# daac-tools/daachorse

Hardware: NVIDIA H100
Metric: input GB/s scanned, find_overlapping_iter, 675k-pat bytewise (higher is better)
Workload: dtype u8

## Files before the change

### daachorse_b200/csrc/dev_scan.cu

```cuda
#include <cuda_runtime.h>

#include <unistd.h>

#include <algorithm>
#include <atomic>
#include <chrono>
#include <cstdio>
#include <cstdlib>
#include <cstring>
#include <memory>
#include <mutex>
#include <string>
#include <vector>

#include "dev_image.h"
#include "host.h"
#include "scan_lane.cuh"

namespace dach {


constexpr int kMaxThreads = 1024;
constexpr int kMaxDevices = 64;
constexpr uint32_t kRootBytes = 1024;
constexpr int64_t kDefaultDfPairs = 1 << 24;

template <int RK>
using SinkOf = typename std::conditional<
    RK == RK_COUNT, CountSink,
    typename std::conditional<
        RK == RK_FIRST || RK == RK_FIRST_STREAM, FirstSink,
        typename std::conditional<RK == RK_HIST, HistSink, typename std::conditional<RK == RK_DF, DfSink, Emitter>::type>::type>::type>::type;

template <bool CHARWISE, int MODE, class SINK>
__device__ __forceinline__ void scan_items(const ScanParams& P) {
    extern __shared__ __align__(16) unsigned char smem_raw[];
    uint32_t* s_root = reinterpret_cast<uint32_t*>(smem_raw);
    uint4* s_hot = reinterpret_cast<uint4*>(smem_raw + kRootBytes);
    for (uint32_t i = threadIdx.x; i < 256; i += blockDim.x) s_root[i] = P.root_table[i];
    for (uint32_t i = threadIdx.x; i < P.hot_n; i += blockDim.x) s_hot[i] = P.rec[i];
    __syncthreads();

    RecView V{P.rec, s_hot, P.hot_n, s_root};
    TextWin T;
    SINK E;
    for (;;) {
        const unsigned long long item = bump_u64(&P.ctrl->next_item);
        if (item >= P.n_items) break;
        const uint64_t o0 = P.offs[item], o1 = P.offs[item + 1];
        const uint32_t len = (uint32_t)(o1 - o0);
        T.open(P.text + o0);
        E.begin((uint32_t)item);
        if (MODE == M_LEFTMOST)
            scan_leftmost<CHARWISE>(P, V, T, E, len);
        else
            scan_standard<CHARWISE, MODE>(P, V, T, E, len);
        E.finish(P);
    }
}

template <bool CHARWISE, int MODE>
__global__ void __launch_bounds__(kMaxThreads, 1) k_scan(ScanParams P) {
    scan_items<CHARWISE, MODE, Emitter>(P);
}
template <bool CHARWISE, int MODE, int RK>
__global__ void __launch_bounds__(kMaxThreads, 1) k_scan_rk(ScanParams P) {
    scan_items<CHARWISE, MODE, SinkOf<RK>>(P);
}


__device__ __forceinline__ uint32_t smem_u32(const void* p) { return (uint32_t)__cvta_generic_to_shared(p); }

__device__ __forceinline__ void mbar_init(uint64_t* bar, uint32_t count) {
    asm volatile("mbarrier.init.shared::cta.b64 [%0], %1;" ::"r"(smem_u32(bar)), "r"(count) : "memory");
    asm volatile("fence.mbarrier_init.release.cluster;" ::: "memory");
}
__device__ __forceinline__ void mbar_expect_tx(uint64_t* bar, uint32_t bytes) {
// ... 83 lines not shown
            if (need) {
                const unsigned long long item = base + __popc(m & ((1u << lane) - 1u));
                if (item < n_items)
                    OPS::begin_item(L, P, Ev, E, item, nullptr);
                else
                    exhausted = true;
            }
        }
        if (!__any_sync(FULL, (L.fl & F_ACTIVE) != 0)) break;
        bool stop = false;
        while (!stop) {
            M::text_topup(L, Ev, nullptr);
            if (M::LEAN) {
#pragma unroll 1
                for (int k = 0; k < M::TOPUP; ++k) (void)M::step(L, Ev, nullptr);
                stop = __any_sync(FULL, (L.fl & (F_ACTIVE | M::IDLE)) == (F_ACTIVE | M::IDLE));
            } else if (M::LAZY) {
                bool waiting = false;
#pragma unroll 1
                for (int k = 0; k < M::TOPUP; ++k) {
                    const bool ok = M::step(L, Ev, nullptr);
                    waiting |= !ok;
                }
                stop = __any_sync(FULL, waiting && (L.fl & F_ACTIVE));
            } else {
#pragma unroll 1
                for (int k = 0; k < M::TOPUP; ++k) {
                    const bool ok = M::step(L, Ev, nullptr);
                    if (__any_sync(FULL, !ok && (L.fl & F_ACTIVE))) {
                        stop = true;
                        break;
                    }
                }
            }
        }
    }
    if constexpr (SINK::KIND == RK_HIST) {
        __syncthreads();
        for (uint32_t i = threadIdx.x; i < P.hist_smem; i += blockDim.x)
            if (E.s_cnt[i]) red_add_u64(P.slot_hist + i, E.s_cnt[i]);
    }
}

template <class M, class LANE, int MAXT, int MINB, bool HOT>
__global__ void __launch_bounds__(MAXT, MINB) k_scan_machine(ScanParams P) {
    if constexpr (M::QLEN)
        scan_machine<M, EventOps<M::ITER>, LANE, EventSink, HOT>(P);
    else
        scan_machine<M, M, LANE, Emitter, HOT>(P);
}
template <class M, class LANE, int MODE, int RK, bool HOT>
__global__ void __launch_bounds__(1024, 1) k_scan_machine_rk(ScanParams P) {
    scan_machine<M, SinkOps<M, MODE, RK>, LANE, SinkOf<RK>, HOT>(P);
}

template <int MODE, int MAXT, bool HOT>
__global__ void __launch_bounds__(MAXT, 1) k_scan_duo(ScanParams P) {
    using M = StdMachine3<MODE>;
    extern __shared__ __align__(128) unsigned char smem_raw[];
    uint4* s_hot = reinterpret_cast<uint4*>(smem_raw);
    QEntry* s_queue = reinterpret_cast<QEntry*>(smem_raw + (HOT ? (size_t)P.hot_entries * 16 : 0));
    __shared__ __align__(8) uint64_t s_bar;
    if (HOT) {
        if (threadIdx.x == 0) mbar_init(&s_bar, 1);
        __syncthreads();
        if (threadIdx.x == 0) {
            const uint32_t hot_bytes = P.hot_entries * 16u;
            mbar_expect_tx(&s_bar, hot_bytes);
            for (uint32_t off = 0; off < hot_bytes; off += 32768u)
                tma_bulk_g2s(reinterpret_cast<unsigned char*>(s_hot) + off, reinterpret_cast<const unsigned char*>(P.crec) + off,
                             min(32768u, hot_bytes - off), &s_bar);
        }
    }
    const StdEnv Ev0{P.crec, s_hot, smem_u32(s_hot), HOT ? P.hot_entries : 0u, P.opos_tab, P.text_end, P.text_lo, P.root_base, P.root_opos ? CF_OUT : 0u,
                     s_queue + threadIdx.x, blockDim.x, 0u, P.mapper, P.mapper_len, ld_u4(P.crec + D_ROOT)};
    StdEnv Ev1 = Ev0;
    Ev1.q = s_queue + (size_t)LANE_Q * blockDim.x + threadIdx.x;
    const unsigned FULL = 0xffffffffu;
    const unsigned lane = threadIdx.x & 31u;
    const unsigned lt = (1u << lane) - 1u;
    Lane3 L0, L1;
    L0.fl = L1.fl = M::IDLE;
    L0.qn = L1.qn = 0;
    Emitter E0, E1;
    E0.begin(0);
    E1.begin(0);
    bool exhausted = false;
    const unsigned long long n_items = P.n_items_dev ? *P.n_items_dev : P.n_items;
    constexpr uint32_t WAIT = F_ACTIVE | F3_STOP;
    if (HOT) mbar_wait(&s_bar, 0);
    for (;;) {
        if (L0.fl & F_ACTIVE) M::drain(L0, Ev0, P, E0);
        if (L1.fl & F_ACTIVE) M::drain(L1, Ev1, P, E1);
        if ((L0.fl & (F_ACTIVE | F_DONE)) == (F_ACTIVE | F_DONE)) {
            E0.finish(P);
            M::finish_item(L0, P);
            L0.fl = M::IDLE;
        }
        if ((L1.fl & (F_ACTIVE | F_DONE)) == (F_ACTIVE | F_DONE)) {
            E1.finish(P);
            M::finish_item(L1, P);
            L1.fl = M::IDLE;
        }
        const bool need0 = !(L0.fl & F_ACTIVE) && !exhausted, need1 = !(L1.fl & F_ACTIVE) && !exhausted;
        const unsigned m0 = __ballot_sync(FULL, need0), m1 = __ballot_sync(FULL, need1);
        if (m0 | m1) {
// ... 614 lines not shown
            }
        if (pinned) cudaFreeHost(pinned);
        pinned = nullptr;
        if (offs_stage) cudaFreeHost(offs_stage);
        offs_stage = nullptr;
        offs_stage_bytes = 0;
        for (int i = 0; i < 4; ++i)
            if (ev[i]) {
                cudaEventDestroy(ev[i]);
                ev[i] = nullptr;
            }
        for (int i = 0; i < 2; ++i)
            if (ev_push[i]) {
                cudaEventDestroy(ev_push[i]);
                ev_push[i] = nullptr;
            }
        if (ev_scanned) cudaEventDestroy(ev_scanned);
        if (ev_placed) cudaEventDestroy(ev_placed);
        ev_scanned = ev_placed = nullptr;
        if (stream) cudaStreamDestroy(stream);
        stream = nullptr;
    }
};

}

struct dach_dev {
    int device = 0;
    bool charwise = false;
    uint8_t match_kind = 0;
    uint32_t n_slots = 0, root_opos = 0, mapper_len = 0, max_pattern_len = 0;
    bool segmentable = false;
    uint32_t n_outputs = 0, max_value = 0, n_cslots = 0;
    size_t image_bytes = 0;
    int sm_count = 0;
    size_t smem_optin = 0;
    uint4* d_rec = nullptr;
    uint4* d_outputs = nullptr;
    uint32_t* d_root = nullptr;
    uint4* d_crec = nullptr;
    uint32_t* d_opos = nullptr;
    uint32_t* d_id_in = nullptr;
    uint32_t* d_id_out = nullptr;
    uint32_t hot_slots = 0;
    uint32_t root_base = 0;
    uint32_t* d_mapper = nullptr;
    void* image_base = nullptr;
    size_t image_alloc = 0;
    std::mutex mu;
    Workspace ws;
    static constexpr int kSlots = 4;
    Workspace slot[kSlots];
    int64_t opt_slice_mib = 64;
    int64_t opt_hot_entries = 6144;
    int64_t opt_hist_smem = 1024;
    int64_t opt_df_pairs = kDefaultDfPairs;
    int64_t opt_slice_ramp = 1;
    int64_t opt_tail_seg = 0;
    int64_t opt_gather_ordered = 1;
    int64_t opt_gather_u = 4;
    int64_t opt_reserve_sms = 0;
    int64_t opt_smem_pad_kib = 0;
    int64_t opt_seg_len = 0;
    int64_t opt_hot_records = 0;
    int64_t opt_threads = 1024;
    int64_t opt_ctas_per_sm = 1;
    int64_t opt_l2_hints = 2;
    int64_t opt_kernel = 3;
    std::atomic<uint64_t> launches{0};
    cudaEvent_t ev_ref = nullptr;
    double last_scan_ms = 0, last_total_ms = 0;
    uint64_t last_h2d = 0, last_d2h = 0;
    DevBuf df_tab[2], df_list[2], df_n, df_acc;
    uint32_t df_mask = 0, df_limit = 0;
    bool df_clean = false;
    uint64_t last_df_windows = 0, last_df_rescans = 0;
    std::atomic<int> refs{1};
};

struct dach_job {
    dach_dev* d = nullptr;
    Workspace W;
    uint64_t out_cap = ~0ull;
};

namespace {

struct DeviceGuard {
    int prev = -1;
    bool ok = false;
    explicit DeviceGuard(int dev) {
        if (cudaGetDevice(&prev) != cudaSuccess) prev = -1;
        ok = cuda_ok(cudaSetDevice(dev), "cudaSetDevice");
        if (!ok) cudaGetLastError();
    }
    ~DeviceGuard() {
        if (prev >= 0) cudaSetDevice(prev);
    }
};

template <bool CW, int MODE>
cudaError_t launch_scan_t(const ScanParams& P, int grid, int threads, size_t smem, cudaStream_t st) {
    static bool attr_done[kMaxDevices] = {};
    int dev = 0;
    cudaGetDevice(&dev);
    if (dev < 0 || dev >= kMaxDevices || !attr_done[dev]) {
        cudaError_t e = cudaFuncSetAttribute(k_scan<CW, MODE>, cudaFuncAttributeMaxDynamicSharedMemorySize, 226 * 1024);
// ... 22 lines not shown
cudaError_t launch_std_modes(int mode, const ScanParams& P, int grid, int threads, size_t smem, cudaStream_t st) {
    switch (mode) {
        case M_FIND: return launch_machine_t<M<M_FIND>, LANE, MAXT, MINB, HOT>(P, grid, threads, smem, st);
        case M_NO_SUFFIX: return launch_machine_t<M<M_NO_SUFFIX>, LANE, MAXT, MINB, HOT>(P, grid, threads, smem, st);
        case M_OVERLAPPING: return launch_machine_t<M<M_OVERLAPPING>, LANE, MAXT, MINB, HOT>(P, grid, threads, smem, st);
    }
    return cudaErrorInvalidValue;
}

cudaError_t launch_std(int which, int mode, const ScanParams& P, int grid, int threads, size_t smem, cudaStream_t st,
                       bool dense) {
    if (which >= 3) {
        if (P.hot_entries)
            return dense ? launch_std_modes<StdMachine3, Lane3, 768, 2, true>(mode, P, grid, threads, smem, st)
                         : launch_std_modes<StdMachine3, Lane3, 1024, 1, true>(mode, P, grid, threads, smem, st);
        return dense ? launch_std_modes<StdMachine3, Lane3, 768, 2, false>(mode, P, grid, threads, smem, st)
                     : launch_std_modes<StdMachine3, Lane3, 1024, 1, false>(mode, P, grid, threads, smem, st);
    }
    if (which == 2)
        return dense ? launch_std_modes<StdMachine2, Lane2, 768, 2, false>(mode, P, grid, threads, smem, st)
                     : launch_std_modes<StdMachine2, Lane2, 1024, 1, false>(mode, P, grid, threads, smem, st);
    return dense ? launch_std_modes<StdMachine, LaneStd, 768, 2, false>(mode, P, grid, threads, smem, st)
                 : launch_std_modes<StdMachine, LaneStd, 1024, 1, false>(mode, P, grid, threads, smem, st);
}

template <int MODE, int MAXT, bool HOT>
cudaError_t launch_duo_t(const ScanParams& P, int grid, int threads, size_t smem, cudaStream_t st) {
    static bool attr_done[kMaxDevices] = {};
    int dev = 0;
    cudaGetDevice(&dev);
    if (dev < 0 || dev >= kMaxDevices || !attr_done[dev]) {
        cudaError_t e = cudaFuncSetAttribute(k_scan_duo<MODE, MAXT, HOT>, cudaFuncAttributeMaxDynamicSharedMemorySize, 226 * 1024);
        if (e != cudaSuccess) return e;
        if (dev >= 0 && dev < kMaxDevices) attr_done[dev] = true;
    }
    k_scan_duo<MODE, MAXT, HOT><<<grid, threads, smem, st>>>(P);
    return cudaGetLastError();
}
template <int MAXT, bool HOT>
cudaError_t launch_duo_m(int mode, const ScanParams& P, int grid, int threads, size_t smem, cudaStream_t st) {
    switch (mode) {
        case M_FIND: return launch_duo_t<M_FIND, MAXT, HOT>(P, grid, threads, smem, st);
        case M_NO_SUFFIX: return launch_duo_t<M_NO_SUFFIX, MAXT, HOT>(P, grid, threads, smem, st);
        case M_OVERLAPPING: return launch_duo_t<M_OVERLAPPING, MAXT, HOT>(P, grid, threads, smem, st);
    }
    return cudaErrorInvalidValue;
}
cudaError_t launch_duo(int mode, const ScanParams& P, int grid, int threads, size_t smem, cudaStream_t st) {
    if (threads > 768)
        return P.hot_entries ? launch_duo_m<1024, true>(mode, P, grid, threads, smem, st) : launch_duo_m<1024, false>(mode, P, grid, threads, smem, st);
    return P.hot_entries ? launch_duo_m<768, true>(mode, P, grid, threads, smem, st) : launch_duo_m<768, false>(mode, P, grid, threads, smem, st);
}

cudaError_t launch_cw(int mode, const ScanParams& P, int grid, int threads, size_t smem, cudaStream_t st) {
    switch (mode) {
        case M_FIND: return launch_machine_t<CwMachine<M_FIND>, LaneCw, 1024, 1, false>(P, grid, threads, smem, st);
        case M_OVERLAPPING: return launch_machine_t<CwMachine<M_OVERLAPPING>, LaneCw, 1024, 1, false>(P, grid, threads, smem, st);
        case M_NO_SUFFIX: return launch_machine_t<CwMachine<M_NO_SUFFIX>, LaneCw, 1024, 1, false>(P, grid, threads, smem, st);
        default: return launch_machine_t<CwMachine<M_LEFTMOST>, LaneCw, 1024, 1, false>(P, grid, threads, smem, st);
    }
}

cudaError_t launch_lm(const ScanParams& P, int grid, int threads, size_t smem, cudaStream_t st) {
    return launch_machine_t<LmMachine, LaneLm, 1024, 1, false>(P, grid, threads, smem, st);
}

cudaError_t launch_scan(bool cw, int mode, const ScanParams& P, int grid, int threads, size_t smem, cudaStream_t st) {
    switch ((cw ? 4 : 0) + mode) {
        case 0: return launch_scan_t<false, M_FIND>(P, grid, threads, smem, st);
        case 1: return launch_scan_t<false, M_OVERLAPPING>(P, grid, threads, smem, st);
        case 2: return launch_scan_t<false, M_NO_SUFFIX>(P, grid, threads, smem, st);
        case 3: return launch_scan_t<false, M_LEFTMOST>(P, grid, threads, smem, st);
        case 4: return launch_scan_t<true, M_FIND>(P, grid, threads, smem, st);
        case 5: return launch_scan_t<true, M_OVERLAPPING>(P, grid, threads, smem, st);
        case 6: return launch_scan_t<true, M_NO_SUFFIX>(P, grid, threads, smem, st);
        case 7: return launch_scan_t<true, M_LEFTMOST>(P, grid, threads, smem, st);
    }
    return cudaErrorInvalidValue;
}

template <class M, class LANE, int MODE, int RK, bool HOT>
cudaError_t launch_rk_t(const ScanParams& P, int grid, int threads, size_t smem, cudaStream_t st) {
    static bool attr_done[kMaxDevices] = {};
    int dev = 0;
    cudaGetDevice(&dev);
    if (dev < 0 || dev >= kMaxDevices || !attr_done[dev]) {
        cudaError_t e = cudaFuncSetAttribute(k_scan_machine_rk<M, LANE, MODE, RK, HOT>, cudaFuncAttributeMaxDynamicSharedMemorySize, 226 * 1024);
        if (e != cudaSuccess) return e;
        if (dev >= 0 && dev < kMaxDevices) attr_done[dev] = true;
    }
    k_scan_machine_rk<M, LANE, MODE, RK, HOT><<<grid, threads, smem, st>>>(P);
    return cudaGetLastError();
}
template <bool CW, int MODE, int RK>
cudaError_t launch_scan_rk_t(const ScanParams& P, int grid, int threads, size_t smem, cudaStream_t st) {
    static bool attr_done[kMaxDevices] = {};
    int dev = 0;
    cudaGetDevice(&dev);
    if (dev < 0 || dev >= kMaxDevices || !attr_done[dev]) {
        cudaError_t e = cudaFuncSetAttribute(k_scan_rk<CW, MODE, RK>, cudaFuncAttributeMaxDynamicSharedMemorySize, 226 * 1024);
        if (e != cudaSuccess) return e;
        if (dev >= 0 && dev < kMaxDevices) attr_done[dev] = true;
    }
    k_scan_rk<CW, MODE, RK><<<grid, threads, smem, st>>>(P);
    return cudaGetLastError();
}
// ... 63 lines not shown
        return DACH_INVALID_ARGUMENT;
    }
    const bool lm = is_leftmost(d->match_kind);
    if ((mode == DACH_LEFTMOST_FIND) != lm) {
        set_error(lm ? "Error: match_kind must be standard." : "Error: match_kind must be leftmost.");
        return DACH_MATCH_KIND_MISMATCH;
    }
    return DACH_OK;
}

bool install_policies(int hints) {
    unsigned long long* d_pol = nullptr;
    unsigned long long h_pol[3] = {0, 0, 0};
    if (!cuda_ok(cudaMalloc(reinterpret_cast<void**>(&d_pol), 24), "cudaMalloc policies")) return false;
    k_make_policies<<<1, 1>>>(d_pol, hints);
    bool ok = cuda_ok(cudaMemcpy(h_pol, d_pol, 24, cudaMemcpyDeviceToHost), "read policies");
    cudaFree(d_pol);
    return ok && cuda_ok(cudaMemcpyToSymbol(c_l2pol, h_pol, 24), "install policies");
}

ScanParams image_params(const dach_dev* d, const uint8_t* d_text, const uint8_t* text_lo, const uint8_t* text_end,
                        const uint64_t* d_offs, uint64_t n) {
    ScanParams P;
    memset(&P, 0, sizeof(P));
    P.rec = d->d_rec;
    P.outputs = d->d_outputs;
    P.root_table = d->d_root;
    P.crec = d->d_crec;
    P.opos_tab = d->d_opos;
    P.root_base = d->root_base;
    P.mapper = d->d_mapper;
    P.mapper_len = d->mapper_len;
    P.n_slots = d->n_slots;
    P.id_in = d->d_id_in;
    P.id_out = d->d_id_out;
    P.root_opos = d->root_opos;
    P.text = d_text;
    P.text_lo = text_lo;
    P.text_end = text_end;
    P.offs = d_offs;
    P.n_items = n;
    return P;
}

size_t plan_smem(const dach_dev* d, ScanParams& P, bool v1, bool std3, int threads, int ctas_per_sm, int queue_sets,
                 uint32_t hist_smem = 0) {
    const size_t smem_budget = std::min<size_t>(d->smem_optin, 226 * 1024) / ctas_per_sm - (ctas_per_sm > 1 ? 1024 : 0);
    size_t smem;
    if (v1) {
        const size_t queues = (size_t)LANE_Q * threads * sizeof(QEntry) * queue_sets + (size_t)hist_smem * 4;
        uint64_t want = 0;
        if (std3 && d->opt_hot_entries != 0 && smem_budget > queues + 512) {
            want = std::min<uint64_t>(d->hot_slots, (smem_budget - queues - 512) / 16);
            if (d->opt_hot_entries > 0) want = std::min<uint64_t>(want, (uint64_t)d->opt_hot_entries);
            want &= ~uint64_t(255);
        }
        smem = (size_t)want * 16 + queues;
        if (d->opt_smem_pad_kib > 0) smem = std::min<size_t>(smem + ((size_t)d->opt_smem_pad_kib << 10), smem_budget);
        P.hot_n = 0;
        P.hot_entries = (uint32_t)want;
    } else {
        uint64_t hot = smem_budget > kRootBytes ? (smem_budget - kRootBytes) / 16 : 0;
        if (d->opt_hot_records >= 0) hot = std::min<uint64_t>(hot, (uint64_t)d->opt_hot_records);
        hot = std::min<uint64_t>(hot, d->n_slots);
        P.hot_n = (uint32_t)hot;
        smem = kRootBytes + (size_t)hot * 16;
    }
    return smem;
}

void enqueue_seg_table(dach_dev* d, Workspace& W, const uint64_t* d_offs, uint64_t n, uint32_t seg_len, uint32_t seg_from,
                       ScanParams& P, cudaStream_t st) {
    unsigned long long* tiles = static_cast<unsigned long long*>(W.tiles.p);
    unsigned long long* seg_first = static_cast<unsigned long long*>(W.seg_first.p);
    const unsigned hb = (unsigned)((n + 255) / 256), hb1 = (unsigned)((n + 1 + 255) / 256);
    const uint64_t nt = (n + kScanTile - 1) / kScanTile;
    uint32_t* nseg = static_cast<uint32_t*>(W.nseg.p);
    k_seg_count<<<hb, 256, 0, st>>>(d_offs, n, seg_len, seg_from, nseg, P.ctrl);
    k_offsets_tile_sums<1><<<(unsigned)nt, kScanThreads, 0, st>>>(nseg, n, tiles);
    k_offsets_scan_tiles<<<1, kScanThreads, 0, st>>>(tiles, nt);
    k_offsets_apply<1><<<(unsigned)nt, kScanThreads, 0, st>>>(nseg, n, tiles, seg_first);
    k_seg_fill<<<hb1, 256, 0, st>>>(seg_first, nseg, n, seg_len, static_cast<uint32_t*>(W.item_hay.p),
                                    static_cast<uint32_t*>(W.item_beg.p), static_cast<unsigned long long*>(W.n_items_dev.p));
    d->launches += 5;
    P.item_hay = static_cast<const uint32_t*>(W.item_hay.p);
    P.item_beg = static_cast<const uint32_t*>(W.item_beg.p);
    P.n_items_dev = static_cast<const unsigned long long*>(W.n_items_dev.p);
    P.seg_len = seg_len;
    P.seg_from = seg_from;
    P.warm = d->max_pattern_len ? d->max_pattern_len - 1 : 0;
}

int enqueue_scan(dach_dev* d, Workspace& W, int mode, const uint8_t* d_text, const uint8_t* text_lo, const uint8_t* text_end,
                 uint64_t text_bytes, const uint64_t* d_offs, uint64_t n, uint64_t cap_matches, cudaStream_t st,
                 uint32_t* d_state_io = nullptr) {
    W.refused = false;
    if (n > 0xfffffff0ull) {
        set_error("too many haystacks in one batch (max 2^32-16)");
        return DACH_INVALID_ARGUMENT;
    }
    if (W.job_open) cudaStreamWaitEvent(st, W.ev_placed, 0);
    W.job_n = n;
    W.job_cap = cap_matches;
    W.job_items = n;
    W.job_seg = false;
    W.job_ordered = false;
    W.job_events = false;
    W.job_stream = st;
    W.job_open = true;
    if (!ensure(W.ctrl, sizeof(ScanCtrl)) || !ensure(W.item_offs, 16)) return DACH_CUDA_ERROR;
    if (!cuda_ok(cudaMemsetAsync(W.ctrl.p, 0, sizeof(ScanCtrl), st), "memset ctrl")) return DACH_CUDA_ERROR;
    cudaEventRecord(W.ev[0], st);
    cudaEventRecord(W.ev[3], st);
    if (n == 0) {
        cudaMemsetAsync(W.item_offs.p, 0, 8, st);
        cudaEventRecord(W.ev[1], st);
        cudaEventRecord(W.ev_scanned, st);
        return DACH_OK;
    }
    int threads = (int)std::min<int64_t>(std::max<int64_t>(d->opt_threads, 32), kMaxThreads);
    threads = (threads / 32) * 32;
    int ctas_per_sm = (int)std::min<int64_t>(std::max<int64_t>(d->opt_ctas_per_sm, 1), 2048 / threads);
    const int free_sms = (int)std::min<int64_t>(std::max<int64_t>(d->opt_reserve_sms, 0), d->sm_count - 1);
    const int grid = (d->sm_count - free_sms) * ctas_per_sm;
    const bool v1 = d->opt_kernel >= 1 && d->d_crec && !(mode == M_FIND && d->root_opos != 0);
    const bool cw_machine = v1 && d->charwise;
    const bool lm_machine = v1 && !d->charwise && mode == M_LEFTMOST;
    const bool std2 = v1 && !d->charwise && mode != M_LEFTMOST && d->opt_kernel >= 2 && d->root_base != 0;
    const bool std3 = std2 && d->opt_kernel >= 3;
    const bool duo = std3 && d->opt_kernel >= 4 && ctas_per_sm == 1;
    const bool events = std3 && !duo;

    if (d_state_io && !std2 && !cw_machine) {
        set_error("stream chunks need a Standard lane machine (find / find_overlapping, at most 2^24 states, bytewise: "
                  "BASE(ROOT) != 0, no empty pattern for find)");
        return DACH_INVALID_ARGUMENT;
    }

    bool seg = v1 && !d->charwise && !d_state_io && (mode == M_OVERLAPPING || mode == M_NO_SUFFIX) && d->opt_seg_len >= 0 && d->segmentable;
    uint32_t seg_len = 0, seg_from = 0;
    uint64_t n_items_max = n;
    if (seg) {
        const uint64_t lanes = (uint64_t)grid * threads;
        const uint64_t warm = d->max_pattern_len ? d->max_pattern_len - 1 : 0;
        const uint64_t floor_len = std::max<uint64_t>(256, 8 * warm);
        uint64_t want;
        uint64_t tail_bytes = text_bytes;
        if (d->opt_seg_len > 0) {
            want = (uint64_t)d->opt_seg_len;
        } else if (d->opt_tail_seg && n >= 4 * lanes && n < 0xffffffffull) {
            const uint64_t n_tail = 2 * lanes;
            seg_from = (uint32_t)(n - n_tail);
            want = std::max(text_bytes / n / 8 + 1, floor_len);
            cudaMemcpyAsync(&W.pinned->tail_offs[0], d_offs + seg_from, 8, cudaMemcpyDeviceToHost, st);
            cudaMemcpyAsync(&W.pinned->tail_offs[1], d_offs + n, 8, cudaMemcpyDeviceToHost, st);
            if (!cuda_ok(cudaStreamSynchronize(st), "read tail size")) return DACH_CUDA_ERROR;
            tail_bytes = W.pinned->tail_offs[1] - W.pinned->tail_offs[0];
        } else {
            want = std::max(text_bytes / (2 * lanes) + 1, floor_len);
        }
        want = (want + 255) & ~uint64_t(255);
        if (want >= text_bytes || want >= (1ull << 31)) {
            seg = false;
        } else {
            seg_len = (uint32_t)want;
            n_items_max = n + tail_bytes / seg_len + 1;
            if (n_items_max > 0xfffffff0ull) seg = false, n_items_max = n;
        }
    }
    const uint64_t n_tiles = (n_items_max + kScanTile - 1) / kScanTile;
    uint64_t pool_blocks64 = cap_matches / BLK_MATCHES + n_items_max + 1024;
    if (pool_blocks64 > 0xffffff00ull) pool_blocks64 = 0xffffff00ull;
    const uint32_t pool_blocks = (uint32_t)pool_blocks64;
    if (!ensure(W.counts, n_items_max * 4) || !ensure(W.tiles, n_tiles * 8) || !ensure(W.item_offs, (n_items_max + 1) * 8) ||
        !ensure(W.pool, (size_t)pool_blocks * BLK_WORDS * 4) || (events && !ensure(W.ev_counts, n_items_max * 4)))
        return DACH_CUDA_ERROR;
    if (seg && (!ensure(W.nseg, n * 4) || !ensure(W.seg_first, (n + 1) * 8) || !ensure(W.item_hay, n_items_max * 4) ||
                !ensure(W.item_beg, n_items_max * 4) || !ensure(W.n_items_dev, 8)))
        return DACH_CUDA_ERROR;

    ScanParams P = image_params(d, d_text, text_lo, text_end, d_offs, n);
    P.counts = static_cast<uint32_t*>(W.counts.p);
    P.ev_counts = events ? static_cast<uint32_t*>(W.ev_counts.p) : nullptr;
    P.pool = static_cast<uint32_t*>(W.pool.p);
    P.pool_blocks = pool_blocks;
    P.ctrl = static_cast<ScanCtrl*>(W.ctrl.p);
    P.state_io = d_state_io;
    const size_t smem = plan_smem(d, P, v1, std3, threads, ctas_per_sm, duo ? 2 : 1);

    unsigned long long* tiles = static_cast<unsigned long long*>(W.tiles.p);
    unsigned long long* item_offs = static_cast<unsigned long long*>(W.item_offs.p);
    k_check_offsets<<<(unsigned)((n + 255) / 256), 256, 0, st>>>(d_offs, n, (uint64_t)(text_end - d_text), P.ctrl);
    ++d->launches;
    if (seg) {
        cudaMemsetAsync(W.counts.p, 0, n_items_max * 4, st);
        if (events) cudaMemsetAsync(W.ev_counts.p, 0, n_items_max * 4, st);
        enqueue_seg_table(d, W, d_offs, n, seg_len, seg_from, P, st);
    }
    cudaEventRecord(W.ev[3], st);
    if (!cuda_ok(cw_machine   ? launch_cw(mode, P, grid, std::min(threads, 1024), smem, st)
                 : lm_machine ? launch_lm(P, grid, std::min(threads, 1024), smem, st)
                 : duo        ? launch_duo(mode, P, grid, threads, smem, st)
                 : v1         ? launch_std(std3 ? 3 : std2 ? 2 : 1, mode, P, grid, threads, smem, st,
                                           ctas_per_sm >= 2 && threads <= 768 && grid % 2 == 0)
                              : launch_scan(d->charwise, mode, P, grid, threads, smem, st),
                 "k_scan launch"))
        return DACH_CUDA_ERROR;
    cudaEventRecord(W.ev[1], st);
    k_offsets_tile_sums<1><<<(unsigned)n_tiles, kScanThreads, 0, st>>>(P.counts, n_items_max, tiles);
    k_offsets_scan_tiles<<<1, kScanThreads, 0, st>>>(tiles, n_tiles);
    k_offsets_apply<1><<<(unsigned)n_tiles, kScanThreads, 0, st>>>(P.counts, n_items_max, tiles, item_offs);
    d->launches += 4;
    const bool ordered = d->opt_gather_ordered >= 2 || (d->opt_gather_ordered == 1 && text_bytes >= (256ull << 20));
    if (ordered) {
        if (!ensure(W.blk_first, (n_items_max + 1) * 8) || !ensure(W.blkmap, (size_t)pool_blocks * 4) || !ensure(W.tiles2, n_tiles * 8))
            return DACH_CUDA_ERROR;
        unsigned long long* tiles2 = static_cast<unsigned long long*>(W.tiles2.p);
        unsigned long long* blk_first = static_cast<unsigned long long*>(W.blk_first.p);
        if (events) {
            k_offsets_tile_sums<BLK_EVENTS><<<(unsigned)n_tiles, kScanThreads, 0, st>>>(P.ev_counts, n_items_max, tiles2);
            k_offsets_scan_tiles<<<1, kScanThreads, 0, st>>>(tiles2, n_tiles);
            k_offsets_apply<BLK_EVENTS><<<(unsigned)n_tiles, kScanThreads, 0, st>>>(P.ev_counts, n_items_max, tiles2, blk_first);
        } else {
            k_offsets_tile_sums<BLK_MATCHES><<<(unsigned)n_tiles, kScanThreads, 0, st>>>(P.counts, n_items_max, tiles2);
            k_offsets_scan_tiles<<<1, kScanThreads, 0, st>>>(tiles2, n_tiles);
            k_offsets_apply<BLK_MATCHES><<<(unsigned)n_tiles, kScanThreads, 0, st>>>(P.counts, n_items_max, tiles2, blk_first);
        }
        k_blk_index<<<d->sm_count * 8, 256, 0, st>>>(P.pool, P.ctrl, pool_blocks, blk_first, static_cast<uint32_t*>(W.blkmap.p));
        d->launches += 4;
    }
    if (!cuda_ok(cudaGetLastError(), "kernel launch")) return DACH_CUDA_ERROR;
    cudaEventRecord(W.ev_scanned, st);
    W.job_items = n_items_max;
    W.job_seg = seg;
    W.job_ordered = ordered;
    W.job_events = events;
    W.job_mode = mode;
    W.job_pool_blocks = pool_blocks;
    return DACH_OK;
}

int enqueue_place(dach_dev* d, Workspace& W, dach_match* d_out, uint64_t out_cap, uint64_t* d_out_offs,
                  const unsigned long long* d_base, bool last, cudaStream_t st, const uint32_t* d_pos_in = nullptr,
                  bool staged = false, bool dma = false, uint64_t h_base = 0, uint64_t h_total = 0) {
    if (!W.job_open) {
        set_error("no scan to place");
        return DACH_INVALID_ARGUMENT;
    }
    if (st != W.job_stream) cudaStreamWaitEvent(st, W.ev_scanned, 0);
    const uint64_t n = W.job_n, n_items = W.job_items;
    const ScanCtrl* ctrl = static_cast<const ScanCtrl*>(W.ctrl.p);
    const unsigned long long* item_offs = static_cast<const unsigned long long*>(W.item_offs.p);
    unsigned long long* offs64 = reinterpret_cast<unsigned long long*>(d_out_offs);
    const int gather_grid = d->sm_count * 8;
    if (n) {
        const uint32_t* pool = static_cast<const uint32_t*>(W.pool.p);
// ... 1375 lines not shown
}

void dach_group_free(dach_group* G) {
    if (!G) return;
    DeviceGuard g(G->device);
    cudaDeviceSynchronize();
    for (int i = 0; i < G->n_ipc; ++i) cudaIpcCloseMemHandle(G->ipc_opened[i]);
    if (G->rank == 0) {
        cudaFree(G->out);
        cudaFree(G->offs);
    }
    cudaFree(G->ctl);
    if (G->pinned) cudaFreeHost(G->pinned);
    if (G->h_vals) cudaFreeHost(G->h_vals);
    delete G;
}

uint64_t dach_dev_kernel_launches(const dach_dev* d) { return d ? d->launches.load() : 0; }
double dach_dev_last_scan_kernel_ms(const dach_dev* d) { return d ? d->last_scan_ms : 0; }
double dach_dev_last_total_ms(const dach_dev* d) { return d ? d->last_total_ms : 0; }
uint64_t dach_dev_last_h2d_bytes(const dach_dev* d) { return d ? d->last_h2d : 0; }
uint64_t dach_dev_last_d2h_bytes(const dach_dev* d) { return d ? d->last_d2h : 0; }

int dach_dev_set_option(dach_dev* d, const char* name, int64_t value) {
    if (!d || !name) return DACH_INVALID_ARGUMENT;
    std::lock_guard<std::mutex> lk(d->mu);
    const std::string k(name);
    if (k == "hot_records")
        d->opt_hot_records = value;
    else if (k == "threads")
        d->opt_threads = value;
    else if (k == "ctas_per_sm")
        d->opt_ctas_per_sm = value;
    else if (k == "kernel")
        d->opt_kernel = value;
    else if (k == "slice_mib")
        d->opt_slice_mib = value;
    else if (k == "seg_len")
        d->opt_seg_len = value;
    else if (k == "slice_ramp")
        d->opt_slice_ramp = value;
    else if (k == "tail_seg")
        d->opt_tail_seg = value;
    else if (k == "gather_ordered")
        d->opt_gather_ordered = value;
    else if (k == "gather_u")
        d->opt_gather_u = value;
    else if (k == "reserve_sms")
        d->opt_reserve_sms = value;
    else if (k == "smem_pad_kib")
        d->opt_smem_pad_kib = value;
    else if (k == "hot_entries")
        d->opt_hot_entries = value;
    else if (k == "hist_smem")
        d->opt_hist_smem = value;
    else if (k == "df_pairs")
        d->opt_df_pairs = value;
    else if (k == "l2_hints") {
        d->opt_l2_hints = value;
        DeviceGuard g(d->device);
        if (!g.ok || !install_policies((int)value)) return DACH_CUDA_ERROR;
    } else {
        set_error("unknown option " + k);
        return DACH_INVALID_ARGUMENT;
    }
    return DACH_OK;
}

}
```

### daachorse_b200/csrc/scan_lane.cuh

```cuda
#pragma once

#include <stdint.h>

#include <type_traits>

#if defined(__CUDACC__)
#define DACH_HD __host__ __device__ __forceinline__
#else
#define DACH_HD inline
#ifndef DACH_EMU_TYPES
#define DACH_EMU_TYPES
struct uint4 {
    uint32_t x, y, z, w;
};
struct uint2 {
    uint32_t x, y;
};
#endif
#endif

#if defined(__CUDA_ARCH__)
#define DACH_SYNCWARP() __syncwarp()
#else
#define DACH_SYNCWARP()
// ... 1646 lines not shown
        L.from = beg;
        L.item = (uint32_t)item;
        L.qn = 0;
        E.begin((uint32_t)item);
        const uint8_t* b0 = block_of(L);
        const uint2 a = ld_text8(b0, Ev.text_end, emu_lo);
        const uint2 n = ld_text8(b0 + 8, Ev.text_end, emu_lo);
        const uint32_t sh = (((uint32_t)(uintptr_t)L.hay + L.pos) & 7u) * 8u;
        const uint64_t cur = (((uint64_t)a.y << 32) | a.x) >> sh;
        L.w0 = (uint32_t)cur;
        L.w1 = (uint32_t)(cur >> 32);
        L.n0 = n.x;
        L.n1 = n.y;
        to_root(L, Ev);
        L.addr = D_ROOT;
        L.fl = F_ACTIVE;
        if (P.state_io) {
            uint32_t st = P.state_io[item];
            if (st != D_ROOT && st < P.n_slots) {
                if (P.id_in) st = P.id_in[st];
                const uint4 x = ld_u4(Ev.glob + st);
                L.r0 = x.x;
                L.nf = x.y;
                L.r2 = x.z;
                L.sig = x.w;
                L.addr = st;
            }
            return;
        }
        if (MODE != M_FIND && (Ev.root_flags & CF_OUT) && beg == 0) {
            QEntry e;
            e.end = 0;
            e.opos = D_ROOT;
            Ev.q[0] = e;
            L.qn = 1;
        }
    }
};


constexpr uint32_t F3_STOP = 0x10u;
constexpr uint32_t F3_LEARN = 0x20u;

struct Lane3 {
    uint32_t hay_lo, hay_hi;
    uint32_t ap, ap_end;
    uint32_t w0, w1, n0, n1;
    uint32_t r0, nf, r2, sig;
    uint32_t addr;
    uint32_t qn, fl, item;
    uint32_t from;
};

DACH_HD uint2 ld_text8_safe(const uint8_t* q, const uint8_t* text_lo, const uint8_t* text_end) {
    uint2 w;
    w.x = w.y = 0;
    if (q >= text_end || q + 8 <= text_lo) return w;
    if (q >= text_lo && q + 8 <= text_end) {
#if defined(__CUDA_ARCH__)
        asm volatile("ld.global.nc.L2::cache_hint.v2.u32 {%0,%1}, [%2], %3;" : "=r"(w.x), "=r"(w.y) : "l"(q), "l"(c_l2pol[1]));
#else
        for (int i = 0; i < 8; ++i) (i < 4 ? w.x : w.y) |= (uint32_t)q[i] << ((i & 3) * 8);
#endif
        return w;
    }
    for (int i = 0; i < 8; ++i) {
        const uint8_t* qi = q + i;
        if (qi >= text_lo && qi < text_end) {
#if defined(__CUDA_ARCH__)
            const uint32_t b = __ldg(qi);
#else
            const uint32_t b = *qi;
#endif
            (i < 4 ? w.x : w.y) |= b << ((i & 3) * 8);
        }
    }
    return w;
}

template <int MODE>
struct StdMachine3 {
    static constexpr int TOPUP = 8;
    static constexpr bool LAZY = true;
    static constexpr bool LEAN = true;
    static constexpr uint32_t IDLE = F3_STOP;
    static constexpr bool QLEN = true;
    static constexpr int ITER = MODE;

    static DACH_HD uint4 fetch(const StdEnv& Ev, uint32_t a) {
#if defined(__CUDA_ARCH__) && defined(DACH_FETCH_GENERIC)
        const uint4* q = a < Ev.hot_n ? Ev.hot + a : Ev.glob + a;
        return *q;
#else
        if (a < Ev.hot_n) {
            DACH_STAT(cache_hits);
#if defined(__CUDA_ARCH__)
            uint4 v;
            asm volatile("ld.shared.v4.u32 {%0,%1,%2,%3}, [%4];" : "=r"(v.x), "=r"(v.y), "=r"(v.z), "=r"(v.w) : "r"(Ev.hot_s + a * 16u));
            return v;
#else
            return Ev.hot[a];
#endif
        }
        return ld_u4(Ev.glob + a);
#endif
    }
    static DACH_HD const uint8_t* block_of(const Lane3& L) {
        const uint64_t hi = (uint64_t)(L.hay_hi + (L.ap < L.hay_lo ? 1u : 0u));
        return reinterpret_cast<const uint8_t*>((uintptr_t)((hi << 32) | (L.ap & ~7u)));
    }
    static DACH_HD void text_topup(Lane3& L, const StdEnv& Ev, const uint8_t* emu_lo) {
        (void)emu_lo;
        if (L.fl & F_NEED_NW) {
            const uint2 n = ld_text8_safe(block_of(L) + 8, Ev.text_lo, Ev.text_end);
            L.n0 = n.x;
            L.n1 = n.y;
            L.fl &= ~F_NEED_NW;
        }
    }
    static DACH_HD void to_root(Lane3& L, const StdEnv& Ev) {
        L.r0 = Ev.root_rec.x;
        L.nf = Ev.root_rec.y;
        L.r2 = Ev.root_rec.z;
        L.sig = Ev.root_rec.w;
        L.addr = D_ROOT;
    }

    static DACH_HD void land(Lane3& L, const StdEnv& Ev) {
        ++L.ap;
        L.w0 = (L.w0 >> 8) | (L.w1 << 24);
        L.w1 >>= 8;
        if ((L.ap & 7u) == 0) {
            L.w0 = L.n0;
            L.w1 = L.n1;
            L.fl |= F_NEED_NW;
        }
        if (L.ap == L.ap_end) L.fl |= F_DONE | F3_STOP;
        if (L.nf & CF_OUT) {
            DACH_STAT(pushes);
            QEntry e;
            e.end = L.ap - L.hay_lo;
            e.opos = MODE == M_OVERLAPPING ? L.addr | (L.r2 << 24) : L.addr;
            Ev.q[L.qn * Ev.q_stride] = e;
            if (++L.qn == (uint32_t)LANE_Q) L.fl |= F3_STOP;
            if (MODE == M_FIND) to_root(L, Ev);
        }
    }

    static DACH_HD uint32_t probe(const Lane3& L, uint32_t& own) {
        const uint32_t c = L.w0 & 0xffu;
        own = (L.sig >> (L.w0 & 31u)) & 1u;
        const uint32_t a = ((own ? L.r0 : L.r2) >> 8) ^ c;
        return (L.fl & F3_STOP) ? 0u : a;
    }
    static DACH_HD void resolve(Lane3& L, const StdEnv& Ev, const uint4& x, uint32_t a, uint32_t own) {
        if (L.fl & (F3_STOP | F3_LEARN)) {
            if (L.fl & F3_STOP) return;
            DACH_STAT(steps);
            DACH_STAT(learns);
            L.nf = x.y;
            L.r2 = x.z;
            L.sig &= ~(1u << (L.w0 & 31u));
            L.fl &= ~F3_LEARN;
            return;
        }
        DACH_STAT(steps);
        DACH_STAT(probes);
        if (((x.x ^ L.w0) & 0xffu) == 0) {
            DACH_STAT(hits);
            L.r0 = x.x;
            L.nf = x.y;
            L.r2 = x.z;
            L.sig = x.w;
            L.addr = a;
            land(L, Ev);
        } else if (own) {
            DACH_STAT(miss_known);
            L.sig &= ~(1u << (L.w0 & 31u));
        } else if (L.nf & CF_FROOT) {
            DACH_STAT(root_stay);
            to_root(L, Ev);
            land(L, Ev);
        } else if (L.nf & CF_F2ROOT) {
            DACH_STAT(miss_f2root);
            L.r2 = Ev.root_base << 8;
            L.nf |= CF_FROOT;
        } else {
            L.r0 = ((L.nf >> 8) ^ (L.w0 & 0xffu)) << 8;
            L.sig |= 1u << (L.w0 & 31u);
            L.fl |= F3_LEARN;
        }
    }
    static DACH_HD bool step(Lane3& L, const StdEnv& Ev, const uint8_t* emu_lo = nullptr) {
        (void)emu_lo;
        if (L.fl & F3_STOP) return false;
        uint32_t own;
        const uint32_t a = probe(L, own);
        const uint4 x = fetch(Ev, a);
        resolve(L, Ev, x, a, own);
        return true;
    }

    static DACH_HD void drain(Lane3& L, const StdEnv& Ev, const ScanParams& P, Emitter& E) {
        for (uint32_t j = 0; j < (uint32_t)LANE_Q; ++j) {
            if (j < L.qn) {
                const QEntry e = Ev.q[j * Ev.q_stride];
                if (e.end >= L.from) {
                    const uint32_t opos = ld_u32(Ev.opos + (e.opos & QSLOT_MASK));
                    if (MODE == M_OVERLAPPING)
                        emit_chain(P, E, opos, e.end);
                    else
                        emit_head(P, E, opos, e.end);
                }
            }
        }
        L.qn = 0;
        if (!(L.fl & F_DONE)) L.fl &= ~F3_STOP;
    }

    static DACH_HD void finish_item(const Lane3& L, const ScanParams& P) {
        if (P.state_io) P.state_io[L.item] = P.id_out ? P.id_out[L.addr] : L.addr;
    }

    static DACH_HD void begin_item(Lane3& L, const ScanParams& P, const StdEnv& Ev, Emitter& E, uint64_t item,
                                   const uint8_t* emu_lo) {
        (void)emu_lo;
        uint64_t hay = item;
        uint32_t beg = 0;
        if (P.item_hay) {
            hay = P.item_hay[item];
            beg = P.item_beg[item];
        }
        const uint64_t o0 = P.offs[hay], o1 = P.offs[hay + 1];
        const uint32_t hay_len = (uint32_t)(o1 - o0);
        const uintptr_t h = (uintptr_t)(P.text + o0);
        L.hay_lo = (uint32_t)h;
        L.hay_hi = (uint32_t)((uint64_t)h >> 32);
        uint32_t start = 0, end = hay_len;
        if (P.item_hay && hay >= P.seg_from) {
            const uint64_t e64 = (uint64_t)beg + P.seg_len;
            if (e64 < hay_len) end = (uint32_t)e64;
            start = beg > P.warm ? beg - P.warm : 0;
        }
        L.ap = L.hay_lo + start;
        L.ap_end = L.hay_lo + end;
        L.from = beg ? beg + 1 : 0;
// ... 94 lines not shown
                const QEntry e = Ev.q[(LANE_Q - 1) * Ev.q_stride];
                if (e.end >= L.from) {
                    emit_head(P, E, ld_u32(Ev.opos + (e.opos & QSLOT_MASK)), e.end);
                    L.fl |= F_DONE | M::IDLE;
                }
            }
            if (!(L.fl & F_DONE)) L.qn = (uint32_t)LANE_Q - 1;
        }
        if (!(L.fl & F_DONE)) L.fl &= ~M::IDLE;
    }
};

template <int MODE>
struct EventOps {
    using M = StdMachine3<MODE>;

    static DACH_HD void begin_item(Lane3& L, const ScanParams& P, const StdEnv& Ev, EventSink& E, uint64_t item,
                                   const uint8_t* emu_lo) {
        Emitter unused;
        M::begin_item(L, P, Ev, unused, item, emu_lo);
        E.begin((uint32_t)item);
    }

    static DACH_HD uint32_t reportable(const Lane3& L, const StdEnv& Ev) {
        uint32_t n = 0;
        for (uint32_t j = 0; j < (uint32_t)LANE_Q; ++j)
            if (j < L.qn && Ev.q[j * Ev.q_stride].end >= L.from) ++n;
        return n;
    }
    static DACH_HD bool need_block(const Lane3& L, const StdEnv& Ev, const EventSink& E) {
        return reportable(L, Ev) > BLK_EVENTS - E.fill;
    }

    static DACH_HD void drain(Lane3& L, const StdEnv& Ev, const ScanParams& P, EventSink& E, uint32_t blk) {
        for (uint32_t j = 0; j < (uint32_t)LANE_Q; ++j) {
            if (j < L.qn) {
                const QEntry e = Ev.q[j * Ev.q_stride];
                if (e.end >= L.from) {
                    if (E.fill == BLK_EVENTS) E.open(P, blk);
                    if (E.blk) st_stream_u2(E.blk + BLK_HDR_WORDS + 2 * E.fill, e.end, e.opos);
                    ++E.fill;
                    ++E.nev;
                    const uint32_t c = E.count + (MODE == M_OVERLAPPING ? qentry_len(P, Ev.opos, e.opos) : 1u);
                    if (c < E.count) count_carry(P);
                    E.count = c;
                }
            }
        }
        L.qn = 0;
        if (!(L.fl & F_DONE)) L.fl &= ~F3_STOP;
    }
};

}
```

Measured before the change: 122.8.

## Add direct-emit scan kernel that writes events inline, freeing queue smem for hot records

Adds a k_scan_direct kernel where each lane writes output events straight into its event block as matches land, instead of pushing them to a shared-memory queue and draining it later. Only the rare case of a full block or an escaped length is deferred through a pending slot. Because the queue is gone, plan_smem can give nearly the whole shared-memory budget to hot trie records, and the new auto hot_entries default does this. A carveout attribute is also set. The risk is more divergent global stores inside the step loop and higher register pressure from the larger per-lane state.

```diff
diff --git a/daachorse_b200/csrc/dev_scan.cu b/daachorse_b200/csrc/dev_scan.cu
--- a/daachorse_b200/csrc/dev_scan.cu
+++ b/daachorse_b200/csrc/dev_scan.cu
@@ -23,6 +23,11 @@
 constexpr int kMaxThreads = 1024;
 constexpr int kMaxDevices = 64;
 constexpr uint32_t kRootBytes = 1024;
+constexpr int64_t kHotAuto = -2;
+constexpr int64_t kHotQueued = 6144;
+constexpr uint32_t kSmemCarveoutStep = 196 * 1024, kSmemPerSmMax = 228 * 1024;
+constexpr uint32_t kDirectSmemBudget = kSmemCarveoutStep - 1024 - 512;
+constexpr int kDirectCarveoutPct = (int)(100ull * kSmemCarveoutStep / kSmemPerSmMax);
 constexpr int64_t kDefaultDfPairs = 1 << 24;
 
 template <int RK>
@@ -212,6 +217,77 @@
 template <class M, class LANE, int MODE, int RK, bool HOT>
 __global__ void __launch_bounds__(1024, 1) k_scan_machine_rk(ScanParams P) {
     scan_machine<M, SinkOps<M, MODE, RK>, LANE, SinkOf<RK>, HOT>(P);
+}
+
+template <int MODE, bool HOT>
+__global__ void __launch_bounds__(1024, 1) k_scan_direct(ScanParams P) {
+    using M = StdMachine3<MODE>;
+    using OPS = DirectOps<MODE>;
+    extern __shared__ __align__(128) unsigned char smem_raw[];
+    uint4* s_hot = reinterpret_cast<uint4*>(smem_raw);
+    __shared__ __align__(8) uint64_t s_bar;
+    if (HOT) {
+        if (threadIdx.x == 0) mbar_init(&s_bar, 1);
+        __syncthreads();
+        if (threadIdx.x == 0) {
+            const uint32_t hot_bytes = P.hot_entries * 16u;
+            mbar_expect_tx(&s_bar, hot_bytes);
+            for (uint32_t off = 0; off < hot_bytes; off += 32768u)
+                tma_bulk_g2s(reinterpret_cast<unsigned char*>(s_hot) + off, reinterpret_cast<const unsigned char*>(P.crec) + off,
+                             min(32768u, hot_bytes - off), &s_bar);
+        }
+    }
+    const StdEnv Ev{P.crec,  s_hot,   smem_u32(s_hot), HOT ? P.hot_entries : 0u, P.opos_tab, P.text_end, P.text_lo, P.root_base, P.root_opos ? CF_OUT : 0u,
+                    nullptr, 0u,      0u,              P.mapper,                 P.mapper_len, ld_u4(P.crec + D_ROOT)};
+    const unsigned FULL = 0xffffffffu;
+    const unsigned lane = threadIdx.x & 31u;
+    Lane3D L;
+    L.fl = M::IDLE;
+    L.qn = 0;
+    L.E.begin(0);
+    bool exhausted = false;
+    const unsigned long long n_items = P.n_items_dev ? *P.n_items_dev : P.n_items;
+    if (HOT) mbar_wait(&s_bar, 0);
+    for (;;) {
+        const bool want = OPS::need_block(L);
+        const unsigned mb = __ballot_sync(FULL, want);
+        uint32_t blk = 0;
+        if (mb) {
+            const int leader = __ffs(mb) - 1;
+            unsigned int b0 = 0;
+            if ((int)lane == leader) b0 = atomicAdd(&P.ctrl->blk_cursor, (unsigned int)__popc(mb));
+            blk = __shfl_sync(FULL, b0, leader) + __popc(mb & ((1u << lane) - 1u));
+        }
+        if (L.fl & F_ACTIVE) OPS::drain(L, Ev, P, blk);
+        if ((L.fl & (F_ACTIVE | F_DONE)) == (F_ACTIVE | F_DONE)) {
+            L.E.finish(P);
+            M::finish_item(L, P);
+            L.fl = M::IDLE;
+        }
+        const bool need = !(L.fl & F_ACTIVE) && !exhausted;
+        const unsigned m = __ballot_sync(FULL, need);
+        if (m) {
+            const int leader = __ffs(m) - 1;
+            unsigned long long base = 0;
+            if ((int)lane == leader) base = atomicAdd(&P.ctrl->next_item, (unsigned long long)__popc(m));
+            base = __shfl_sync(FULL, base, leader);
+            if (need) {
+                const unsigned long long item = base + __popc(m & ((1u << lane) - 1u));
+                if (item < n_items)
+                    OPS::begin_item(L, P, Ev, item);
+                else
+                    exhausted = true;
+            }
+        }
+        if (!__any_sync(FULL, (L.fl & F_ACTIVE) != 0)) break;
+        bool stop = false;
+        while (!stop) {
+            M::text_topup(L, Ev, nullptr);
+#pragma unroll 1
+            for (int k = 0; k < M::TOPUP; ++k) (void)M::step(L, Ev, nullptr);
+            stop = __any_sync(FULL, (L.fl & (F_ACTIVE | F3_STOP)) == (F_ACTIVE | F3_STOP));
+        }
+    }
 }
 
 template <int MODE, int MAXT, bool HOT>
@@ -932,7 +1008,8 @@
     static constexpr int kSlots = 4;
     Workspace slot[kSlots];
     int64_t opt_slice_mib = 64;
-    int64_t opt_hot_entries = 6144;
+    int64_t opt_hot_entries = kHotAuto;
+    int64_t opt_event_queue = 0;
     int64_t opt_hist_smem = 1024;
     int64_t opt_df_pairs = kDefaultDfPairs;
     int64_t opt_slice_ramp = 1;
@@ -1061,6 +1138,35 @@
     return P.hot_entries ? launch_duo_m<768, true>(mode, P, grid, threads, smem, st) : launch_duo_m<768, false>(mode, P, grid, threads, smem, st);
 }
 
+template <int MODE, bool HOT>
+cudaError_t launch_direct_t(const ScanParams& P, int grid, int threads, size_t smem, cudaStream_t st) {
+    static bool attr_done[kMaxDevices] = {};
+    int dev = 0;
+    cudaGetDevice(&dev);
+    if (dev < 0 || dev >= kMaxDevices || !attr_done[dev]) {
+        cudaError_t e = cudaFuncSetAttribute(k_scan_direct<MODE, HOT>, cudaFuncAttributeMaxDynamicSharedMemorySize, 226 * 1024);
+        if (e == cudaSuccess)
+            e = cudaFuncSetAttribute(k_scan_direct<MODE, HOT>, cudaFuncAttributePreferredSharedMemoryCarveout, kDirectCarveoutPct);
+        if (e != cudaSuccess) return e;
+        if (dev >= 0 && dev < kMaxDevices) attr_done[dev] = true;
+    }
+    k_scan_direct<MODE, HOT><<<grid, threads, smem, st>>>(P);
+    return cudaGetLastError();
+}
+cudaError_t launch_direct(int mode, const ScanParams& P, int grid, int threads, size_t smem, cudaStream_t st) {
+    switch (mode) {
+        case M_FIND:
+            return P.hot_entries ? launch_direct_t<M_FIND, true>(P, grid, threads, smem, st) : launch_direct_t<M_FIND, false>(P, grid, threads, smem, st);
+        case M_NO_SUFFIX:
+            return P.hot_entries ? launch_direct_t<M_NO_SUFFIX, true>(P, grid, threads, smem, st)
+                                 : launch_direct_t<M_NO_SUFFIX, false>(P, grid, threads, smem, st);
+        case M_OVERLAPPING:
+            return P.hot_entries ? launch_direct_t<M_OVERLAPPING, true>(P, grid, threads, smem, st)
+                                 : launch_direct_t<M_OVERLAPPING, false>(P, grid, threads, smem, st);
+    }
+    return cudaErrorInvalidValue;
+}
+
 cudaError_t launch_cw(int mode, const ScanParams& P, int grid, int threads, size_t smem, cudaStream_t st) {
     switch (mode) {
         case M_FIND: return launch_machine_t<CwMachine<M_FIND>, LaneCw, 1024, 1, false>(P, grid, threads, smem, st);
@@ -1230,7 +1336,8 @@
         uint64_t want = 0;
         if (std3 && d->opt_hot_entries != 0 && smem_budget > queues + 512) {
             want = std::min<uint64_t>(d->hot_slots, (smem_budget - queues - 512) / 16);
-            if (d->opt_hot_entries > 0) want = std::min<uint64_t>(want, (uint64_t)d->opt_hot_entries);
+            const int64_t hot = d->opt_hot_entries != kHotAuto ? d->opt_hot_entries : queue_sets ? kHotQueued : kDirectSmemBudget / 16;
+            if (hot > 0) want = std::min<uint64_t>(want, (uint64_t)hot);
             want &= ~uint64_t(255);
         }
         smem = (size_t)want * 16 + queues;
@@ -1308,6 +1415,7 @@
     const bool std3 = std2 && d->opt_kernel >= 3;
     const bool duo = std3 && d->opt_kernel >= 4 && ctas_per_sm == 1;
     const bool events = std3 && !duo;
+    const bool direct = events && ctas_per_sm == 1 && d->opt_event_queue == 0;
 
     if (d_state_io && !std2 && !cw_machine) {
         set_error("stream chunks need a Standard lane machine (find / find_overlapping, at most 2^24 states, bytewise: "
@@ -1364,7 +1472,7 @@
     P.pool_blocks = pool_blocks;
     P.ctrl = static_cast<ScanCtrl*>(W.ctrl.p);
     P.state_io = d_state_io;
-    const size_t smem = plan_smem(d, P, v1, std3, threads, ctas_per_sm, duo ? 2 : 1);
+    const size_t smem = plan_smem(d, P, v1, std3, threads, ctas_per_sm, duo ? 2 : direct ? 0 : 1);
 
     unsigned long long* tiles = static_cast<unsigned long long*>(W.tiles.p);
     unsigned long long* item_offs = static_cast<unsigned long long*>(W.item_offs.p);
@@ -1379,7 +1487,8 @@
     if (!cuda_ok(cw_machine   ? launch_cw(mode, P, grid, std::min(threads, 1024), smem, st)
                  : lm_machine ? launch_lm(P, grid, std::min(threads, 1024), smem, st)
                  : duo        ? launch_duo(mode, P, grid, threads, smem, st)
-                 : v1         ? launch_std(std3 ? 3 : std2 ? 2 : 1, mode, P, grid, threads, smem, st,
+                 : direct     ? launch_direct(mode, P, grid, threads, smem, st)
+                 : v1        ? launch_std(std3 ? 3 : std2 ? 2 : 1, mode, P, grid, threads, smem, st,
                                            ctas_per_sm >= 2 && threads <= 768 && grid % 2 == 0)
                               : launch_scan(d->charwise, mode, P, grid, threads, smem, st),
                  "k_scan launch"))
@@ -2861,6 +2970,8 @@
         d->opt_smem_pad_kib = value;
     else if (k == "hot_entries")
         d->opt_hot_entries = value;
+    else if (k == "event_queue")
+        d->opt_event_queue = value;
     else if (k == "hist_smem")
         d->opt_hist_smem = value;
     else if (k == "df_pairs")
diff --git a/daachorse_b200/csrc/scan_lane.cuh b/daachorse_b200/csrc/scan_lane.cuh
--- a/daachorse_b200/csrc/scan_lane.cuh
+++ b/daachorse_b200/csrc/scan_lane.cuh
@@ -1722,6 +1722,13 @@
     uint32_t from;
 };
 
+constexpr uint32_t F3_PEND = 0x40u;
+constexpr uint32_t F3_CARRY = 0x80u;
+struct Lane3D : Lane3 {
+    EventSink E;
+    uint32_t pend_end, pend_slot;
+};
+
 DACH_HD uint2 ld_text8_safe(const uint8_t* q, const uint8_t* text_lo, const uint8_t* text_end) {
     uint2 w;
     w.x = w.y = 0;
@@ -1796,7 +1803,7 @@
         L.addr = D_ROOT;
     }
 
-    static DACH_HD void land(Lane3& L, const StdEnv& Ev) {
+    static DACH_HD void consume(Lane3& L) {
         ++L.ap;
         L.w0 = (L.w0 >> 8) | (L.w1 << 24);
         L.w1 >>= 8;
@@ -1806,6 +1813,10 @@
             L.fl |= F_NEED_NW;
         }
         if (L.ap == L.ap_end) L.fl |= F_DONE | F3_STOP;
+    }
+
+    static DACH_HD void land(Lane3& L, const StdEnv& Ev) {
+        consume(L);
         if (L.nf & CF_OUT) {
             DACH_STAT(pushes);
             QEntry e;
@@ -1816,6 +1827,30 @@
             if (MODE == M_FIND) to_root(L, Ev);
         }
     }
+    static DACH_HD void land(Lane3D& L, const StdEnv& Ev) {
+        consume(L);
+        if (L.nf & CF_OUT) {
+            DACH_STAT(pushes);
+            const uint32_t end = L.ap - L.hay_lo;
+            if (end >= L.from) {
+                const uint32_t slot = MODE == M_OVERLAPPING ? L.addr | (L.r2 << 24) : L.addr;
+                const uint32_t len = MODE == M_OVERLAPPING ? L.r2 & 0xffu : 1u;
+                if (L.E.fill < BLK_EVENTS && len != QLEN_ESCAPE) {
+                    if (L.E.blk) st_stream_u2(L.E.blk + BLK_HDR_WORDS + 2 * L.E.fill, end, slot);
+                    ++L.E.fill;
+                    ++L.E.nev;
+                    const uint32_t c = L.E.count + len;
+                    if (c < L.E.count) L.fl |= F3_CARRY;
+                    L.E.count = c;
+                } else {
+                    L.pend_end = end;
+                    L.pend_slot = slot;
+                    L.fl |= F3_PEND | F3_STOP;
+                }
+            }
+            if (MODE == M_FIND) to_root(L, Ev);
+        }
+    }
 
     static DACH_HD uint32_t probe(const Lane3& L, uint32_t& own) {
         const uint32_t c = L.w0 & 0xffu;
@@ -1823,7 +1858,8 @@
         const uint32_t a = ((own ? L.r0 : L.r2) >> 8) ^ c;
         return (L.fl & F3_STOP) ? 0u : a;
     }
-    static DACH_HD void resolve(Lane3& L, const StdEnv& Ev, const uint4& x, uint32_t a, uint32_t own) {
+    template <class LANE>
+    static DACH_HD void resolve(LANE& L, const StdEnv& Ev, const uint4& x, uint32_t a, uint32_t own) {
         if (L.fl & (F3_STOP | F3_LEARN)) {
             if (L.fl & F3_STOP) return;
             DACH_STAT(steps);
@@ -1861,7 +1897,8 @@
             L.fl |= F3_LEARN;
         }
     }
-    static DACH_HD bool step(Lane3& L, const StdEnv& Ev, const uint8_t* emu_lo = nullptr) {
+    template <class LANE>
+    static DACH_HD bool step(LANE& L, const StdEnv& Ev, const uint8_t* emu_lo = nullptr) {
         (void)emu_lo;
         if (L.fl & F3_STOP) return false;
         uint32_t own;
@@ -2062,4 +2099,41 @@
     }
 };
 
-}
+template <int MODE>
+struct DirectOps {
+    using M = StdMachine3<MODE>;
+
+    static DACH_HD void begin_item(Lane3D& L, const ScanParams& P, const StdEnv& Ev, uint64_t item) {
+        QEntry root;
+        StdEnv Ev1 = Ev;
+        Ev1.q = &root;
+        Emitter unused;
+        M::begin_item(L, P, Ev1, unused, item, nullptr);
+        L.E.begin((uint32_t)item);
+        if (L.qn) {
+            L.pend_end = root.end;
+            L.pend_slot = root.opos;
+            L.fl |= F3_PEND | F3_STOP;
+            L.qn = 0;
+        }
+    }
+    static DACH_HD bool need_block(const Lane3D& L) { return (L.fl & F3_PEND) && L.E.fill == BLK_EVENTS; }
+
+    static DACH_HD void drain(Lane3D& L, const StdEnv& Ev, const ScanParams& P, uint32_t blk) {
+        EventSink& E = L.E;
+        if (L.fl & F3_PEND) {
+            if (E.fill == BLK_EVENTS) E.open(P, blk);
+            if (E.blk) st_stream_u2(E.blk + BLK_HDR_WORDS + 2 * E.fill, L.pend_end, L.pend_slot);
+            ++E.fill;
+            ++E.nev;
+            const uint32_t c = E.count + (MODE == M_OVERLAPPING ? qentry_len(P, Ev.opos, L.pend_slot) : 1u);
+            if (c < E.count) count_carry(P);
+            E.count = c;
+        }
+        if (L.fl & F3_CARRY) count_carry(P);
+        L.fl &= ~(F3_PEND | F3_CARRY);
+        if (!(L.fl & F_DONE)) L.fl &= ~F3_STOP;
+    }
+};
+
+}
```

Measured after the change: 137.9 (median of 6 runs). +12.2%, better.
